# meuleman/epilogos

Measured on AMD Instinct MI355X. Metric: Mbins scored/sec (S1, 18-state, 833 biosamples), higher is better.
Workload: dtype u8

## Files before the change

epilogos_amd/csrc/epg_common.h:

```cpp
#pragma once
#include <hip/hip_runtime.h>
#include <stdarg.h>
#include <stdint.h>
#include <stdio.h>

#include <type_traits>

#include "epilogos_amd.h"

typedef unsigned int u32;
typedef unsigned long long u64;
typedef unsigned short u16;

namespace epg {

int fail(int code, const char* fmt, ...);
int num_cus();

#ifdef EPILOGOS_BUILD_EXPERIMENTS
#include <stdlib.h>
static inline const char* exp_env(const char* name) { return getenv(name); }
#else
static inline const char* exp_env(const char*) { return nullptr; }
#endif

enum Force { FORCE_NULL_SEQ = 0, FORCE_S3_SCORE_BINS, FORCE_S3_CONTRACTION, FORCE_S3_HIST_LDS, FORCE_K1_BLOCKS_PER_CU, FORCE_CUS, FORCE_COUNT };
extern int g_force[FORCE_COUNT];

#define EPG_HIP(expr)                                                                         \
    do {                                                                                      \
        hipError_t _e = (expr);                                                               \
        if (_e != hipSuccess)                                                                 \
            return epg::fail(EPG_ERR_HIP, "%s failed: %s", #expr, hipGetErrorString(_e));     \
    } while (0)

#define EPG_LAUNCH_CHECK(name)                                                                \
    do {                                                                                      \
        hipError_t _e = hipGetLastError();                                                    \
        if (_e != hipSuccess)                                                                 \
            return epg::fail(EPG_ERR_HIP, "launch of %s failed: %s", name, hipGetErrorString(_e)); \
    } while (0)

static inline int64_t align_up(int64_t x, int64_t a) { return (x + a - 1) / a * a; }

template <int DEFAULT, typename F>
static inline auto with_constant(int, F&& f) {
    return f(std::integral_constant<int, DEFAULT>{});
}
template <int DEFAULT, int V, int... VS, typename F>
static inline auto with_constant(int v, F&& f) {
    if (v == V) return f(std::integral_constant<int, V>{});
    return with_constant<DEFAULT, VS...>(v, f);
}

int64_t s1_ws_bytes(int64_t R, int N, int S);
int grid_for_tiles(long R);
long fast_rows(long R, int N, long ldx);
int64_t s2_table_bytes(int maxc, int S);
int64_t s3_ws_bytes(int64_t R, int N, int S);
int64_t s3_xt_bytes(int64_t R, int N);
int transpose_states(const char* X, int64_t R, int32_t N, int64_t ldx, int32_t S, char* XT, int64_t Rp, int shift, int bad, int* dirty,
                     hipStream_t st);
int64_t s3_gemm_ws_bytes(int64_t R, int N, int S);
int64_t s3_gemm_ws_min_bytes(int64_t R, int N, int S);
int hist_s3_gemm(const char* X, int64_t R, int32_t N, int64_t ldx, int32_t S, int32_t* counts, void* ws, int64_t ws_bytes, hipStream_t st);
bool s3_lanes_ok(int N, int S);
int64_t s3_lanes_ws_bytes(int64_t R, int N, int S);
int score_s3_lanes(const int8_t* X8, int64_t R, int32_t N, int64_t ldx, int32_t S, const float* q, double* out64, float* out32, void* ws,
                   int64_t ws_bytes, hipStream_t st);
int wide_hist_s2_from_binhist(const uint16_t* H, const uint16_t* H2, int64_t R, int32_t S, int64_t* counts, hipStream_t st);
int wide_score_s2_from_hist(const uint16_t* H, int64_t R, int32_t S, int64_t perms, const float* q, double* out64, float* out32, hipStream_t st);
int wide_hist_s3(const int8_t* X, int64_t R, int32_t N, int64_t ldx, int32_t S, int32_t* counts, hipStream_t st);
int wide_score_s3(const int8_t* X, int64_t R, int32_t N, int64_t ldx, int32_t S, const float* q, double* out64, float* out32, void* ws,
                  int64_t ws_bytes, hipStream_t st);

struct DynLds {
    unsigned long long done = 0;
};
static inline hipError_t ensure_dyn_lds(DynLds& a, const void* kernel, int bytes) {
    int dev = 0;
    hipError_t e = hipGetDevice(&dev);
    if (e != hipSuccess) return e;
    const unsigned long long bit = 1ull << (dev & 63);
    if (__atomic_load_n(&a.done, __ATOMIC_ACQUIRE) & bit) return hipSuccess;
    e = hipFuncSetAttribute(kernel, hipFuncAttributeMaxDynamicSharedMemorySize, bytes);
    if (e == hipSuccess) __atomic_fetch_or(&a.done, bit, __ATOMIC_RELEASE);
    return e;
}

static inline int tile_rows(int64_t row_bytes) {
    int tr = 64;
    while (tr > 8 && 4 * tr * row_bytes > 65536) tr >>= 1;
    return tr;
}

__device__ __forceinline__ u32 bfi(u32 m, u32 a, u32 b) { return (a & m) | (b & ~m); }

__device__ __forceinline__ uint4 ld16(const char* p) {
    uint4 v;
    __builtin_memcpy(&v, p, 16);
    return v;
}

__device__ __forceinline__ u32 quad_sum(u32 v) {
    v += (u32)__builtin_amdgcn_update_dpp(0, (int)v, 0xB1, 0xf, 0xf, false);
    v += (u32)__builtin_amdgcn_update_dpp(0, (int)v, 0x4E, 0xf, 0xf, false);
    return v;
}

__device__ __forceinline__ void store_staged(const char* lds, char* dst, int nbytes, int lane) {
    const int nchunks = nbytes >> 4;
    for (int c = lane; c < nchunks; c += 64)
        *reinterpret_cast<uint4*>(dst + 16 * c) = *reinterpret_cast<const uint4*>(lds + 16 * c);
    const int tail0 = nchunks << 4;
    for (int o = tail0 + 4 * lane; o + 4 <= nbytes; o += 256)
        *reinterpret_cast<u32*>(dst + o) = *reinterpret_cast<const u32*>(lds + o);
    if ((nbytes & 2) && lane == 0) *reinterpret_cast<u16*>(dst + nbytes - 2) = *reinterpret_cast<const u16*>(lds + nbytes - 2);
}

typedef u32 epg_u32x4 __attribute__((ext_vector_type(4)));
__device__ __forceinline__ void store_staged_nt(const char* lds, char* dst, int nbytes, int lane) {
    const int nchunks = nbytes >> 4;
    for (int c = lane; c < nchunks; c += 64)
        __builtin_nontemporal_store(*reinterpret_cast<const epg_u32x4*>(lds + 16 * c), reinterpret_cast<epg_u32x4*>(dst + 16 * c));
    const int tail0 = nchunks << 4;
    for (int o = tail0 + 4 * lane; o + 4 <= nbytes; o += 256)
        __builtin_nontemporal_store(*reinterpret_cast<const u32*>(lds + o), reinterpret_cast<u32*>(dst + o));
    if ((nbytes & 2) && lane == 0) *reinterpret_cast<u16*>(dst + nbytes - 2) = *reinterpret_cast<const u16*>(lds + nbytes - 2);
}

__device__ __forceinline__ double kl_term(double p, double q) {
    if (q == 0.0) return 0.0;
    const double r = p / q;
    if (!(r > 0.0)) return 0.0;
    return p * log2(r);
}

__device__ __forceinline__ float s3_table_entry(float qv, float obs) {
    if (qv == 0.0f) return 0.0f;
    const float r = __fdiv_rn(obs, qv);
    if (!(r > 0.0f)) return 0.0f;
#ifdef EPG_S3_TABLE_LOG2F
    return obs * log2f(r);
#else
    return __fmul_rn(obs, (float)log2((double)r));
#endif
}

}
```

epilogos_amd/csrc/epg_count.h:

```cpp
#pragma once
#include "epg_common.h"
#include "epg_parts.h"

namespace epg {

#define EPG_B3(a, b, c, tt) ((u32)__builtin_amdgcn_bitop3_b32((int)(a), (int)(b), (int)(c), (tt)))

__device__ __forceinline__ u32 sel(u32 m, u32 x, u32 y) { return EPG_B3(m, x, y, 0xCA); }

__device__ __forceinline__ u32 dbl(u32 x) {
    u32 r;
    asm("v_add_u32 %0, %1, %1" : "=v"(r) : "v"(x));
    return r;
}

__device__ __forceinline__ void bit_planes(const u32 (&w)[8], u32 (&P)[5]) {
    const u32 n0 = sel(0x0f0f0f0fu, w[0], w[1] << 4);
    const u32 n1 = sel(0x0f0f0f0fu, w[2], w[3] << 4);
    const u32 n2 = sel(0x0f0f0f0fu, w[4], w[5] << 4);
    const u32 n3 = sel(0x0f0f0f0fu, w[6], w[7] << 4);
    const u32 m0 = sel(0x33333333u, n0, n1 << 2), m1 = sel(0x33333333u, n2, n3 << 2);
    const u32 r0 = sel(0xccccccccu, n1, n0 >> 2), r1 = sel(0xccccccccu, n3, n2 >> 2);
    P[0] = sel(0x55555555u, m0, dbl(m1)); P[1] = sel(0xaaaaaaaau, m1, m0 >> 1);
    P[2] = sel(0x55555555u, r0, dbl(r1)); P[3] = sel(0xaaaaaaaau, r1, r0 >> 1);
    const u32 c00 = sel(0x10101010u, w[0], dbl(w[4])), c01 = sel(0x10101010u, w[1], dbl(w[5]));
    const u32 c10 = sel(0x10101010u, w[2], dbl(w[6])), c11 = sel(0x10101010u, w[3], dbl(w[7]));
    const u32 d0 = sel(0x30303030u, c00, c10 << 2), d1 = sel(0x30303030u, c01, c11 << 2);
    P[4] = sel(0xf0f0f0f0u, d1, d0 >> 4);
}

__device__ __forceinline__ void low_three(const u32 (&P)[5], u32 (&L)[8]) {
    L[0] = EPG_B3(P[0], P[1], P[2], 0x01); L[1] = EPG_B3(P[0], P[1], P[2], 0x10); L[2] = EPG_B3(P[0], P[1], P[2], 0x04); L[3] = EPG_B3(P[0], P[1], P[2], 0x40);
    L[4] = EPG_B3(P[0], P[1], P[2], 0x02); L[5] = EPG_B3(P[0], P[1], P[2], 0x20); L[6] = EPG_B3(P[0], P[1], P[2], 0x08); L[7] = EPG_B3(P[0], P[1], P[2], 0x80);
}

__device__ __forceinline__ u32 indicator(const u32 (&L)[8], const u32 (&P)[5], int s) {
    switch (s >> 3) {
        case 0: return EPG_B3(L[s & 7], P[3], P[4], 0x10);
        case 1: return EPG_B3(L[s & 7], P[3], P[4], 0x40);
        case 2: return EPG_B3(L[s & 7], P[3], P[4], 0x20);
        default: return EPG_B3(L[s & 7], P[3], P[4], 0x80);
    }
}

template <int S>
__device__ __forceinline__ void count_group(const u32 (&w)[8], u32 (&cnt)[S]) {
    u32 P[5], L[8];
    bit_planes(w, P);
    low_three(P, L);
#pragma unroll
    for (int s = 0; s < S; ++s) cnt[s] += (u32)__builtin_popcount(indicator(L, P, s));
}

struct RowGeom {
    int chunks;
    int last;
    u32 tail[4];
};

__device__ __forceinline__ RowGeom make_geom(int N) {
    RowGeom g;
    g.chunks = (N + 15) >> 4;
    g.last = g.chunks - 1;
    const int t = N - 16 * g.last;
#pragma unroll
    for (int d = 0; d < 4; ++d) {
        int v = t - 4 * d;
        v = v < 0 ? 0 : (v > 4 ? 4 : v);
        g.tail[d] = v == 4 ? 0u : (0xffffffffu << (8 * v));
    }
    return g;
}

template <bool MAYBE_TAIL>
__device__ __forceinline__ void load_slot(const char* rowp, int i, int j, const RowGeom& g, u32* w) {
    const int c = 4 * i + j;
    if (!MAYBE_TAIL) {
        const uint4 v = ld16(rowp + 16 * c);
        w[0] = v.x; w[1] = v.y; w[2] = v.z; w[3] = v.w;
    } else {
        const int cc = c < g.last ? c : g.last;
        const uint4 v = ld16(rowp + 16 * cc);
        const u32 inv = c > g.last ? 0xffffffffu : 0u;
        const bool is_last = c == g.last;
        w[0] = v.x | inv | (is_last ? g.tail[0] : 0u);
        w[1] = v.y | inv | (is_last ? g.tail[1] : 0u);
        w[2] = v.z | inv | (is_last ? g.tail[2] : 0u);
        w[3] = v.w | inv | (is_last ? g.tail[3] : 0u);
    }
}

template <bool MAYBE_TAIL>
__device__ __forceinline__ void load_group(const char* rowp, int t, int j, const RowGeom& g, u32 (&w)[8]) {
    load_slot<MAYBE_TAIL>(rowp, 2 * t, j, g, &w[0]);
    load_slot<MAYBE_TAIL>(rowp, 2 * t + 1, j, g, &w[4]);
}

template <int NG>
__device__ __forceinline__ void load_groups(const char* rowp, int j, const RowGeom& g, u32 (&w)[NG][8]) {
#pragma unroll
    for (int t = 0; t < NG; ++t) {
        if (t < NG - 1) load_group<false>(rowp, t, j, g, w[t]);
        else load_group<true>(rowp, t, j, g, w[t]);
    }
}

template <int NC, typename Group>
__device__ __forceinline__ void for_each_group(const char* rowp, int j, const RowGeom& g, u32 (&cnt)[NC], Group group) {
    const int ngroups = (g.chunks + 7) >> 3;
    for (int t0 = 0; t0 < ngroups; t0 += 4) {
        u32 w[4][8];
#pragma unroll
        for (int k = 0; k < 4; ++k) {
            const int t = t0 + k;
            if (t < ngroups - 1) load_group<false>(rowp, t, j, g, w[k]);
            else if (t == ngroups - 1) load_group<true>(rowp, t, j, g, w[k]);
        }
#pragma unroll
        for (int k = 0; k < 4; ++k)
            if (t0 + k < ngroups) group(t0 + k, w[k], cnt);
    }
}

template <int S, int NG>
__device__ __forceinline__ void count_row(const char* rowp, int j, const RowGeom& g, u32 (&cnt)[S]) {
    if constexpr (NG > 0) {
        u32 w[NG][8];
        load_groups<NG>(rowp, j, g, w);
#pragma unroll
        for (int t = 0; t < NG; ++t) count_group<S>(w[t], cnt);
    } else {
        for_each_group(rowp, j, g, cnt, [](int, const u32 (&w)[8], u32 (&c)[S]) { count_group<S>(w, c); });
    }
}

template <int S, int NG>
struct CountRow {
    __device__ __forceinline__ void operator()(const char* rowp, int j, const RowGeom& g, u32 (&cnt)[S]) const { count_row<S, NG>(rowp, j, g, cnt); }
};

template <int S, typename Count, typename Epilogue, typename Finish>
__device__ __forceinline__ void super_tile(const char* __restrict__ X, long R, long ldx, const RowGeom& g, long lst, int j, int b, Count&& count,
                                           Epilogue&& epilogue, Finish&& finish) {
#pragma unroll
    for (int half = 0; half < 2; ++half) {
        const long row = lst * 32 + half * 16 + b;
        const bool valid = row < R;
        u32 cnt[S];
#pragma unroll
        for (int s = 0; s < S; ++s) cnt[s] = 0;
        count(X + (valid ? row : R - 1) * ldx, j, g, cnt);
        epilogue(half, row, valid, cnt);
    }
    const long row0 = lst * 32;
    finish(lst, row0, (int)(R - row0 < 32 ? R - row0 : 32));
}

template <int S, int NG, int NW = 4, typename Epilogue, typename Finish, typename Count = CountRow<S, NG>>
__device__ __forceinline__ void tile_loop(const char* __restrict__ X, long R, int N, long ldx, Epilogue&& epilogue, Finish&& finish,
                                          Count&& count = Count()) {
    const int lane = threadIdx.x & 63;
    const int wave = __builtin_amdgcn_readfirstlane(threadIdx.x >> 6);
    const int j = lane & 3, b = lane >> 2;
    const RowGeom g = make_geom(N);
    const long nsuper = (R + 31) >> 5;
    for (long st = (long)blockIdx.x * NW + wave; st < nsuper; st += (long)gridDim.x * NW)
        super_tile<S>(X, R, ldx, g, st, j, b, count, epilogue, finish);
}

constexpr int KH_MAXP = 48;
struct KhParts {
    const char* x[KH_MAXP];
    u16* h[KH_MAXP];
    long rows[KH_MAXP];
    long ldx[KH_MAXP];
    long t0[KH_MAXP + 1];
    int n_cols[KH_MAXP];
    int n;
};

template <int S, int NG, int NW = 4, typename Enter, typename Epilogue, typename Finish>
__device__ __forceinline__ void tile_loop_parts(const KhParts& pt, Enter&& enter, Epilogue&& epilogue, Finish&& finish) {
    const int lane = threadIdx.x & 63;
    const int wave = __builtin_amdgcn_readfirstlane(threadIdx.x >> 6);
    const int j = lane & 3, b = lane >> 2;
    const long nsuper = pt.t0[pt.n];
    PartCursor at;
    int part = -1;
    const char* X = nullptr;
    long R = 0, ldx = 0, base = 0;
    RowGeom g = make_geom(16);
    for (long st = (long)blockIdx.x * NW + wave; st < nsuper; st += (long)gridDim.x * NW) {
        at.advance(pt.t0, st, 32);
        if (at.part != part) {
            part = at.part;
            X = pt.x[part];
            R = pt.rows[part];
            ldx = pt.ldx[part];
            base = pt.t0[part];
            g = make_geom(pt.n_cols[part]);
            enter(part);
        }
        super_tile<S>(X, R, ldx, g, st - base, j, b, CountRow<S, NG>(), epilogue, finish);
    }
}

template <int S>
__device__ __forceinline__ void pack_reduce(const u32 (&cnt)[S], u32 (&d)[(S + 1) / 2]) {
#pragma unroll
    for (int m = 0; m < (S + 1) / 2; ++m) {
        const u32 hi = 2 * m + 1 < S ? cnt[2 * m + 1] : 0u;
        d[m] = quad_sum(cnt[2 * m] | (hi << 16));
    }
}

__device__ __forceinline__ u32 sel4(u32 x0, u32 x1, u32 x2, u32 x3, int j) {
    const u32 lo = (j & 1) ? x1 : x0;
    const u32 hi = (j & 1) ? x3 : x2;
    return (j & 2) ? hi : lo;
}

template <int ND>
__device__ __forceinline__ u32 quad_state_count(const u32 (&d)[ND], int k, int j) {
    const u32 lo = d[2 * k], hi = 2 * k + 1 < ND ? d[2 * k + 1] : 0u;
    const u32 v = (j & 2) ? hi : lo;
    return (j & 1) ? v >> 16 : v & 0xffffu;
}

template <int S, bool WHOLE_DWORDS>
__device__ __forceinline__ void stage_hist_row(char* srow, const u32 (&d)[(S + 1) / 2], int j, int Sout) {
    constexpr int ND = (S + 1) / 2;
    if constexpr (WHOLE_DWORDS) {
        static_assert((S & 1) == 0, "whole dwords need an even row");
#pragma unroll
        for (int k = 0; k < (ND + 3) / 4; ++k) {
            const u32 v = sel4(d[4 * k], 4 * k + 1 < ND ? d[4 * k + 1] : 0u, 4 * k + 2 < ND ? d[4 * k + 2] : 0u, 4 * k + 3 < ND ? d[4 * k + 3] : 0u, j);
            if (4 * k + j < ND) *reinterpret_cast<u32*>(srow + 4 * (4 * k + j)) = v;
        }
    } else {
#pragma unroll
        for (int k = 0; k < (S + 3) / 4; ++k) {
            const u32 c = quad_state_count(d, k, j);
            if (4 * k + j < Sout) *reinterpret_cast<u16*>(srow + 2 * (4 * k + j)) = (u16)c;
        }
    }
}

template <int S>
struct StateTotals {
    static constexpr int ND = (S + 1) / 2;
    u32 accp[ND];
    int since, flush_every;
    __device__ __forceinline__ void init(int nmax) {
#pragma unroll
        for (int m = 0; m < ND; ++m) accp[m] = 0;
        flush_every = 65535 / nmax > 1 ? 65535 / nmax - 1 : 1;
        since = 0;
    }
    __device__ __forceinline__ void flush(u64* s_cnt, int j) {
        if (j == 0) {
#pragma unroll
            for (int m = 0; m < ND; ++m) {
                const u32 lo = accp[m] & 0xffffu, hi = accp[m] >> 16;
                if (lo) atomicAdd(&s_cnt[2 * m], (u64)lo);
                if (hi) atomicAdd(&s_cnt[2 * m + 1], (u64)hi);
            }
        }
#pragma unroll
        for (int m = 0; m < ND; ++m) accp[m] = 0;
        since = 0;
    }
    __device__ __forceinline__ void add(const u32 (&d)[ND], bool valid, u64* s_cnt, int j) {
#pragma unroll
        for (int m = 0; m < ND; ++m) accp[m] += valid ? d[m] : 0u;
        if (++since >= flush_every) flush(s_cnt, j);
    }
    __device__ __forceinline__ void commit(u64* s_cnt, int j, u64* __restrict__ counts, int Sout) {
        flush(s_cnt, j);
        __syncthreads();
        if ((int)threadIdx.x < Sout && s_cnt[threadIdx.x]) atomicAdd(&counts[threadIdx.x], s_cnt[threadIdx.x]);
    }
};

}
```

epilogos_amd/csrc/epg_s1.hip:

```cpp
#include "epg_count.h"
#include "epg_paircount.h"

#include <stdlib.h>
#include <string.h>

namespace epg {

constexpr int K1P_LD = 17;

template <int SC, bool FULL, bool PAIRS, typename Loop>
__device__ __forceinline__ void bin_hist_body(int Sout_, u64* __restrict__ counts, int nmax, u64* __restrict__ counts2, Loop&& loop) {
    constexpr int S = SC;
    constexpr int ND = (S + 1) / 2;
    const int Sout = FULL ? S : Sout_;
    const int ROWB = 2 * Sout;
    __shared__ u64 s_cnt[S + 1];
    __shared__ __attribute__((aligned(16))) char s_stage[4][32 * 2 * S];
    constexpr int PG = (S + 2) / 3, PSP = 3 * PG, PROLES = PG * (PG + 1) / 2, PSLICE = PROLES <= 64 ? 64 / PROLES : 1;
    static_assert(!PAIRS || (FULL && PROLES <= 64), "the pair counts need a compile-time row width and at most 64 block roles");
    __shared__ u32 s_pair[PAIRS ? 4 * PSP * K1P_LD : 1];
    __shared__ u64 s_c2[PAIRS ? S * S : 1];
    const int lane = threadIdx.x & 63, wave = threadIdx.x >> 6;
    const int j = lane & 3, b = lane >> 2;
    if (threadIdx.x <= S) s_cnt[threadIdx.x] = 0;
    if (PAIRS) {
        for (int e = threadIdx.x; e < S * S; e += 256) s_c2[e] = 0;
        for (int e = threadIdx.x; e < 4 * PSP * K1P_LD; e += 256) s_pair[e] = 0;
    }
    __syncthreads();
    u16* H = nullptr;
    int pgi = -1, pgj = 0, pkq = 0;
    u64 pacc[PAIRS ? 9 : 1], prs[PAIRS ? 3 : 1];
    if (PAIRS) {
        const int role = lane < PROLES * PSLICE ? lane / PSLICE : -1;
        pkq = lane % PSLICE;
        if (role >= 0) pair_role(role, PG, pgi, pgj);
#pragma unroll
        for (int c = 0; c < 9; ++c) pacc[c] = 0;
#pragma unroll
        for (int c = 0; c < 3; ++c) prs[c] = 0;
    }
    auto pair_counts = [&](const char* stage, int rows) {
        u32* sp = s_pair + wave * PSP * K1P_LD;
        const u16* raw = reinterpret_cast<const u16*>(stage);
        __builtin_amdgcn_wave_barrier();
        for (int e = lane; e < S * 16; e += 64) {
            const int i = e >> 4, k = e & 15;
            const u32 lo = 2 * k < rows ? raw[(2 * k) * S + i] : 0u, hi = 2 * k + 1 < rows ? raw[(2 * k + 1) * S + i] : 0u;
            sp[i * K1P_LD + k] = lo | (hi << 16);
        }
        __builtin_amdgcn_wave_barrier();
        if (pgi >= 0) {
            u32 part[9], ps[3];
            pair_tile_dot(sp + 3 * pgi * K1P_LD, sp + 3 * pgj * K1P_LD, K1P_LD, pkq, 16, PSLICE, pgi == pgj, part, ps);
#pragma unroll
            for (int c = 0; c < 9; ++c) pacc[c] += part[c];
#pragma unroll
            for (int c = 0; c < 3; ++c) prs[c] += ps[c];
        }
        __builtin_amdgcn_wave_barrier();
    };

    StateTotals<S> totals;
    totals.init(nmax);

    auto enter = [&](u16* Hpart) { H = Hpart; };
    auto epilogue = [&](int half, long row, bool valid, u32 (&cnt)[S]) {
        u32 d[ND];
        pack_reduce<S>(cnt, d);
        if (counts) totals.add(d, valid, s_cnt, j);
        if (H) stage_hist_row<S, FULL && (S & 1) == 0>(&s_stage[wave][(half * 16 + b) * ROWB], d, j, Sout);
    };
    auto finish = [&](long st, long row0, int rows) {
        if (H) store_staged(s_stage[wave], reinterpret_cast<char*>(H) + row0 * ROWB, rows * ROWB, lane);
        if constexpr (PAIRS) pair_counts(s_stage[wave], rows);
    };
    loop(enter, epilogue, finish);

    if (counts) totals.commit(s_cnt, j, counts, Sout);
    if constexpr (PAIRS) {
        if (pgi >= 0) pair_fold(pacc, prs, pgi, pgj, S, s_c2);
        pair_commit(s_c2, S, counts2);
    }
}

template <int SC, int NG, bool FULL>
__global__ __launch_bounds__(256) void k_bin_hist(const char* __restrict__ X, long R, int N, long ldx, int Sout_,
                                                   u16* __restrict__ H, u64* __restrict__ counts) {
    bin_hist_body<SC, FULL, false>(Sout_, counts, N, nullptr, [&](auto&& enter, auto&& epilogue, auto&& finish) {
        enter(H);
        tile_loop<SC, NG>(X, R, N, ldx, epilogue, finish);
    });
}

template <int SC, int NG>
__global__ __launch_bounds__(256) void k_bin_hist_s2(const char* __restrict__ X, long R, int N, long ldx, u16* __restrict__ H,
                                                      u64* __restrict__ counts, u64* __restrict__ counts2) {
    bin_hist_body<SC, true, true>(SC, counts, N, counts2, [&](auto&& enter, auto&& epilogue, auto&& finish) {
        enter(H);
        tile_loop<SC, NG>(X, R, N, ldx, epilogue, finish);
    });
}

template <int SC, int NG, bool FULL>
__global__ __launch_bounds__(256) void k_bin_hist_parts(const KhParts pt, int Sout_, u64* __restrict__ counts, int nmax) {
    bin_hist_body<SC, FULL, false>(Sout_, counts, nmax, nullptr, [&](auto&& enter, auto&& epilogue, auto&& finish) {
        tile_loop_parts<SC, NG>(pt, [&](int part) { enter(pt.h[part]); }, epilogue, finish);
    });
}

__global__ __launch_bounds__(256) void k_bin_hist_safe(const char* __restrict__ X, long row_begin, long row_end, int N,
                                                        long ldx, int S, u16* __restrict__ H, u64* __restrict__ counts, int mask = 31) {
    __shared__ u32 s_h[4][128];
    const int lane = threadIdx.x & 63, wave = threadIdx.x >> 6;
    for (long row = row_begin + (long)blockIdx.x * 4 + wave; row < row_end; row += (long)gridDim.x * 4) {
        for (int s = lane; s < S; s += 64) s_h[wave][s] = 0;
        __builtin_amdgcn_wave_barrier();
        const char* rp = X + row * ldx;
        for (int n = lane; n < N; n += 64) {
            const int v = (unsigned char)rp[n] & mask;
            if (v < S) atomicAdd(&s_h[wave][v], 1u);
        }
        __builtin_amdgcn_wave_barrier();
        for (int s = lane; s < S; s += 64) {
            const u32 c = s_h[wave][s];
            if (H) H[row * S + s] = (u16)c;
            if (counts && c) atomicAdd(&counts[s], (u64)c);
        }
        __builtin_amdgcn_wave_barrier();
    }
}

__global__ void k_s1_table(const float* __restrict__ q, int N, int S, double* __restrict__ T64, float* __restrict__ T32) {
    const long e = (long)blockIdx.x * blockDim.x + threadIdx.x;
    if (e >= (long)(N + 1) * S) return;
    const int c = (int)(e / S), s = (int)(e % S);
    const double p = (double)c / (double)N;
    const double v = kl_term(p, (double)q[s]);
    T64[e] = v;
    T32[e] = (float)v;
}

template <int S, int NG, typename OT>
__global__ __launch_bounds__(256) void k_score_s1(const char* __restrict__ X, long R, int N, long ldx,
                                                   const OT* __restrict__ T, OT* __restrict__ out) {
    constexpr int ND = (S + 1) / 2;
    constexpr int ROWB = S * (int)sizeof(OT);
    __shared__ __attribute__((aligned(16))) char s_stage[4][32 * ROWB];
    const int lane = threadIdx.x & 63, wave = threadIdx.x >> 6;
    const int j = lane & 3, b = lane >> 2;
    auto epilogue = [&](int half, long row, bool valid, u32 (&cnt)[S]) {
        u32 d[ND];
        pack_reduce<S>(cnt, d);
        OT* srow = reinterpret_cast<OT*>(&s_stage[wave][(half * 16 + b) * ROWB]);
#pragma unroll
        for (int k = 0; k < (S + 3) / 4; ++k) {
            const u32 c = quad_state_count(d, k, j);
            const int s = 4 * k + j;
            if (s < S) srow[s] = (c && valid) ? T[(long)c * S + s] : (OT)0;
        }
    };
    auto finish = [&](long st, long row0, int rows) {
        store_staged_nt(s_stage[wave], reinterpret_cast<char*>(out) + row0 * ROWB, rows * ROWB, lane);
    };
    tile_loop<S, NG>(X, R, N, ldx, epilogue, finish);
}

template <typename OT, bool LDS_T>
__global__ __launch_bounds__(LDS_T ? 1024 : 256) void k_score_s1_from_hist(const u16* __restrict__ H, long total, int S,
                                                                             const OT* __restrict__ Tg, int nent, OT* __restrict__ out,
                                                                             u64* __restrict__ zero_counts, int rev) {
    extern __shared__ __attribute__((aligned(16))) char smem_t[];
    if (zero_counts && blockIdx.x == 0 && (int)threadIdx.x < S) zero_counts[threadIdx.x] = 0;
    const OT* T = Tg;
    if (LDS_T) {
        OT* Ts = reinterpret_cast<OT*>(smem_t);
        for (int e = threadIdx.x; e < nent; e += blockDim.x) Ts[e] = Tg[e];
        __syncthreads();
        T = Ts;
    }
    const u32 cmax = (u32)(nent / S - 1);
    const long nquads = total >> 2;
    const long stride = (long)gridDim.x * blockDim.x;
    long qd = (long)blockIdx.x * blockDim.x + threadIdx.x;
    const long qtop = nquads - 1, qsgn = rev ? -1 : 1, qoff = rev ? qtop : 0;
    for (; qd + 3 * stride < nquads; qd += 4 * stride) {
        uint2 h[4];
#pragma unroll
        for (int u = 0; u < 4; ++u) h[u] = *reinterpret_cast<const uint2*>(H + 4 * (qoff + qsgn * (qd + u * stride)));
#pragma unroll
        for (int u = 0; u < 4; ++u) {
            const long e0 = 4 * (qoff + qsgn * (qd + u * stride));
            int s = (int)(e0 % S);
            const u32 c[4] = {h[u].x & 0xffffu, h[u].x >> 16, h[u].y & 0xffffu, h[u].y >> 16};
            OT v[4];
#pragma unroll
            for (int k = 0; k < 4; ++k) {
                v[k] = c[k] - 1u < cmax ? T[(long)c[k] * S + s] : (OT)0;
                s = s + 1 == S ? 0 : s + 1;
            }
            if constexpr (sizeof(OT) == 4) {
                typedef float v4f_nt __attribute__((ext_vector_type(4)));
                const v4f_nt vv = {(float)v[0], (float)v[1], (float)v[2], (float)v[3]};
                __builtin_nontemporal_store(vv, reinterpret_cast<v4f_nt*>(out + e0));
            } else {
                typedef double v2d_nt __attribute__((ext_vector_type(2)));
                const v2d_nt lo = {(double)v[0], (double)v[1]}, hi = {(double)v[2], (double)v[3]};
                __builtin_nontemporal_store(lo, reinterpret_cast<v2d_nt*>(out + e0));
                __builtin_nontemporal_store(hi, reinterpret_cast<v2d_nt*>(out + e0 + 2));
            }
        }
    }
    for (; qd < nquads; qd += stride) {
        const long e0 = 4 * (qoff + qsgn * qd);
        int s = (int)(e0 % S);
        for (int k = 0; k < 4; ++k) {
            const u32 c = H[e0 + k];
            out[e0 + k] = c - 1u < cmax ? T[(long)c * S + s] : (OT)0;
            s = s + 1 == S ? 0 : s + 1;
        }
    }
    if (blockIdx.x == 0 && threadIdx.x < (total & 3)) {
        const long e = (nquads << 2) + threadIdx.x;
        const u32 c = H[e];
        out[e] = c - 1u < cmax ? T[(long)c * S + (int)(e % S)] : (OT)0;
    }
}

template <typename IT>
__global__ __launch_bounds__(256) void k_sum_int(const IT* __restrict__ C, long n, long long* __restrict__ total) {
    long long acc = 0;
    for (long i = (long)blockIdx.x * blockDim.x + threadIdx.x; i < n; i += (long)gridDim.x * blockDim.x) acc += (long long)C[i];
    for (int off = 32; off > 0; off >>= 1) acc += __shfl_down(acc, off);
    __shared__ long long s_part[4];
    if ((threadIdx.x & 63) == 0) s_part[threadIdx.x >> 6] = acc;
    __syncthreads();
    if (threadIdx.x == 0) {
        const long long t = s_part[0] + s_part[1] + s_part[2] + s_part[3];
        if (t) atomicAdd(reinterpret_cast<u64*>(total), (u64)t);
    }
}

template <typename IT>
__global__ __launch_bounds__(256) void k_normalise(const IT* __restrict__ C, long n, const long long* __restrict__ total,
                                                    float* __restrict__ q) {
    const double tot = (double)(*total);
    for (long i = (long)blockIdx.x * blockDim.x + threadIdx.x; i < n; i += (long)gridDim.x * blockDim.x)
        q[i] = (float)((double)C[i] / tot);
}

template <typename IT>
__global__ __launch_bounds__(256) void k_normalise_small(const IT* __restrict__ C, int n, float* __restrict__ q) {
    __shared__ long long s_part[4];
    long long acc = 0;
    for (int i = threadIdx.x; i < n; i += 256) acc += (long long)C[i];
    for (int off = 32; off > 0; off >>= 1) acc += __shfl_down(acc, off);
    if ((threadIdx.x & 63) == 0) s_part[threadIdx.x >> 6] = acc;
    __syncthreads();
    const double tot = (double)(s_part[0] + s_part[1] + s_part[2] + s_part[3]);
    for (int i = threadIdx.x; i < n; i += 256) q[i] = (float)((double)C[i] / tot);
}

static int blocks_per_cu() { return g_force[FORCE_K1_BLOCKS_PER_CU] > 0 ? g_force[FORCE_K1_BLOCKS_PER_CU] : 2; }
int grid_for_tiles(long R) {
    const long nsuper = (R + 31) >> 5;
    long blocks = (nsuper + 3) / 4;
    const long cap = (long)num_cus() * blocks_per_cu();
    if (blocks > cap) {
        const long iters = (nsuper + cap * 4 - 1) / (cap * 4);
        blocks = (nsuper + iters * 4 - 1) / (iters * 4);
    }
    if (blocks < 1) blocks = 1;
    return (int)blocks;
}

template <typename F>
static void with_count_core(int S, int ng, F&& f) {
    if (S == 15 || S == 18 || S == 25)
        with_constant<25, 15, 18>(S, [&](auto sc) {
            with_constant<0, 1, 2, 3, 4, 5, 6, 7, 8>(ng, [&](auto NG) { f(sc, NG, std::true_type{}); });
        });
    else
        with_constant<31, 15, 18, 25>(S < 15 ? 15 : S < 18 ? 18 : S < 25 ? 25 : 31,
                                      [&](auto sc) { f(sc, std::integral_constant<int, 0>{}, std::false_type{}); });
}

long fast_rows(long R, int N, long ldx) {
    const long chunks = (N + 15) / 16;
    const long over = 16 * chunks - ldx;
    if (over <= 0) return R;
    const long unsafe = (over + ldx - 1) / ldx;
    return R > unsafe ? R - unsafe : 0;
}

extern "C" int epg_bin_hist(const int8_t* X8, int64_t R, int32_t N, int64_t ldx, int32_t S, uint16_t* H, int64_t* counts, void* stream) {
    hipStream_t st = (hipStream_t)stream;
    if (R < 0 || N < 1 || ldx < N || S < 1) return fail(EPG_ERR_INVALID_ARG, "bin_hist: bad shape R=%lld N=%d ldx=%lld S=%d", (long long)R, N, (long long)ldx, S);
    if (S > 127) return fail(EPG_ERR_UNSUPPORTED, "bin_hist: S=%d > 127 (states are int8)", S);
    if (N > 65535) return fail(EPG_ERR_UNSUPPORTED, "bin_hist: N=%d > 65535 (uint16 per-bin counts)", N);
    if (R == 0) return EPG_OK;
    if (!X8) return fail(EPG_ERR_INVALID_ARG, "bin_hist: X is NULL");
    if (H && (reinterpret_cast<uintptr_t>(H) & 15)) return fail(EPG_ERR_INVALID_ARG, "bin_hist: H must be 16-byte aligned");
    const char* X = reinterpret_cast<const char*>(X8);
    u64* cnt = reinterpret_cast<u64*>(counts);
    if (S > 31) {
        hipLaunchKernelGGL(k_bin_hist_safe, dim3((unsigned)((R + 3) / 4 < num_cus() * 32L ? (R + 3) / 4 : num_cus() * 32L)), dim3(256), 0, st, X, 0L,
                           (long)R, N, ldx, S, H, cnt, 255);
        EPG_LAUNCH_CHECK("k_bin_hist_safe");
        return EPG_OK;
    }
    const long Rf = fast_rows(R, N, ldx);
    if (Rf > 0) {
        with_count_core(S, (N + 127) / 128, [&](auto SC, auto NG, auto MODEL) {
            hipLaunchKernelGGL((k_bin_hist<SC, NG, MODEL && (SC & 1) == 0>), dim3(grid_for_tiles(Rf)), dim3(256), 0, st, X, Rf, N, ldx, S, H, cnt);
        });
        EPG_LAUNCH_CHECK("k_bin_hist");
    }
    if (Rf < R) {
        hipLaunchKernelGGL(k_bin_hist_safe, dim3((unsigned)((R - Rf + 3) / 4 < 1024 ? (R - Rf + 3) / 4 : 1024)), dim3(256), 0, st, X, Rf, (long)R, N, ldx, S, H, cnt);
        EPG_LAUNCH_CHECK("k_bin_hist_safe");
    }
    return EPG_OK;
}

extern "C" int epg_bin_hist_s2(const int8_t* X8, int64_t R, int32_t N, int64_t ldx, int32_t S, uint16_t* H, int64_t* counts, int64_t* counts2,
                               void* stream) {
    hipStream_t st = (hipStream_t)stream;
    if (!H || !counts2) return fail(EPG_ERR_INVALID_ARG, "bin_hist_s2: H and counts2 are required");
    const bool fused = (S == 15 || S == 18 || S == 25) && R > 0 && N >= 1 && N <= 1024 && ldx >= N && X8 &&
                       !(reinterpret_cast<uintptr_t>(H) & 15) && fast_rows(R, N, ldx) == R;
    if (!fused) {
        int rc = epg_bin_hist(X8, R, N, ldx, S, H, counts, stream);
        if (rc) return rc;
        return epg_hist_s2_from_binhist(H, R, S, counts2, stream);
    }
    const char* X = reinterpret_cast<const char*>(X8);
    u64* c1 = reinterpret_cast<u64*>(counts);
    u64* c2 = reinterpret_cast<u64*>(counts2);
    with_constant<25, 18, 15>(S, [&](auto SC) {
        with_constant<8, 1, 2, 3, 4, 5, 6, 7>((N + 127) / 128, [&](auto NG) {
            hipLaunchKernelGGL((k_bin_hist_s2<decltype(SC)::value, NG>), dim3(grid_for_tiles(R)), dim3(256), 0, st, X, R, N, ldx, H, c1, c2);
        });
    });
    EPG_LAUNCH_CHECK("k_bin_hist_s2");
    return EPG_OK;
}

extern "C" int epg_bin_hist_parts(int32_t nparts, const int8_t* const* X, const int64_t* R, const int32_t* N, const int64_t* ldx, int32_t S,
                                  uint16_t* const* H, int64_t* counts, void* stream) {
    hipStream_t st = (hipStream_t)stream;
    if (nparts < 0 || (nparts && (!X || !R || !N || !ldx))) return fail(EPG_ERR_INVALID_ARG, "bin_hist_parts: NULL argument array");
    if (S < 1 || S > 127) return fail(EPG_ERR_UNSUPPORTED, "bin_hist_parts: S=%d outside 1..127", S);
    for (int p = 0; p < nparts; ++p) {
        if (R[p] < 0 || (R[p] && (N[p] < 1 || ldx[p] < N[p]))) return fail(EPG_ERR_INVALID_ARG, "bin_hist_parts: bad shape of part %d", p);
        if (R[p] && N[p] > 65535) return fail(EPG_ERR_UNSUPPORTED, "bin_hist_parts: N=%d > 65535 (uint16 per-bin counts)", N[p]);
        if (R[p] && !X[p]) return fail(EPG_ERR_INVALID_ARG, "bin_hist_parts: X of part %d is NULL", p);
        if (H && H[p] && (reinterpret_cast<uintptr_t>(H[p]) & 15)) return fail(EPG_ERR_INVALID_ARG, "bin_hist_parts: H of part %d must be 16-byte aligned", p);
    }
    if (S > 31) {
        for (int p = 0; p < nparts; ++p) {
            const int rc = epg_bin_hist(X[p], R[p], N[p], ldx[p], S, H ? H[p] : nullptr, counts, stream);
            if (rc) return rc;
        }
        return EPG_OK;
    }
    u64* cnt = reinterpret_cast<u64*>(counts);
    for (int p = 0; p < nparts; ++p) {
        const long Rf = R[p] ? fast_rows(R[p], N[p], ldx[p]) : 0;
        if (Rf == R[p]) continue;
        hipLaunchKernelGGL(k_bin_hist_safe, dim3((unsigned)((R[p] - Rf + 3) / 4 < 1024 ? (R[p] - Rf + 3) / 4 : 1024)), dim3(256), 0, st,
                           reinterpret_cast<const char*>(X[p]), Rf, (long)R[p], N[p], (long)ldx[p], S, H ? H[p] : nullptr, cnt);
        EPG_LAUNCH_CHECK("k_bin_hist_safe");
    }
    auto cls = [](int n) { const int ng = (n + 127) / 128; return ng <= 8 ? ng : 0; };
    for (int c = 0; c <= 8; ++c) {
        for (int p0 = 0; p0 < nparts;) {
            KhParts pt;
            int nmax = 1;
            p0 = pack_parts(pt, p0, nparts, 32, [&](int p) { return R[p] && cls(N[p]) == c ? fast_rows(R[p], N[p], ldx[p]) : 0L; },
                            [&](int k, int p) {
                                pt.x[k] = reinterpret_cast<const char*>(X[p]); pt.h[k] = H ? H[p] : nullptr;
                                pt.ldx[k] = ldx[p]; pt.n_cols[k] = N[p];
                                if (N[p] > nmax) nmax = N[p];
                            });
            if (pt.n == 0) break;
            with_count_core(S, c, [&](auto SC, auto NG, auto) {
                hipLaunchKernelGGL((k_bin_hist_parts<SC, NG, (NG > 0 && (SC & 1) == 0)>), dim3(grid_for_tiles(pt.t0[pt.n] * 32)), dim3(256), 0, st, pt, S,
                                   cnt, nmax);
            });
            EPG_LAUNCH_CHECK("k_bin_hist_parts");
        }
    }
    return EPG_OK;
}

static int64_t s1_table_bytes(int N, int S) { return align_up((int64_t)(N + 1) * S * 8, 256) + align_up((int64_t)(N + 1) * S * 4, 256); }

int64_t s1_ws_bytes(int64_t R, int N, int S) {
    return s1_table_bytes(N, S) + 256 + align_up(R * S * 2, 256);
}

static int build_s1_table(const float* q, int N, int S, void* ws, double** T64, float** T32, hipStream_t st) {
    *T64 = reinterpret_cast<double*>(ws);
    *T32 = reinterpret_cast<float*>(reinterpret_cast<char*>(ws) + align_up((int64_t)(N + 1) * S * 8, 256));
    const long n = (long)(N + 1) * S;
    hipLaunchKernelGGL(k_s1_table, dim3((int)((n + 255) / 256)), dim3(256), 0, st, q, N, S, *T64, *T32);
    EPG_LAUNCH_CHECK("k_s1_table");
    return EPG_OK;
}
static int check_score_from_hist_args(const uint16_t* H, const double* out64, const float* out32) {
    if ((reinterpret_cast<uintptr_t>(H) & 7) != 0) return fail(EPG_ERR_INVALID_ARG, "score_s1_from_binhist: H must be 8-byte aligned");
    if ((out32 && (reinterpret_cast<uintptr_t>(out32) & 15)) || (out64 && (reinterpret_cast<uintptr_t>(out64) & 15)))
        return fail(EPG_ERR_INVALID_ARG, "score_s1_from_binhist: outputs must be 16-byte aligned");
    return EPG_OK;
}

template <typename OT>
static int launch_score_s1_from_hist_t(const uint16_t* H, long total, int32_t S, const OT* T, int nent, OT* out, u64* zero_counts, hipStream_t st) {
    const size_t tbytes = (size_t)nent * sizeof(OT);
    const int rev = 1;
    if (tbytes <= 150 * 1024) {
        const int per_cu = tbytes <= 75 * 1024 ? 2 : 1;
        long nb = (total / 4 + 4095) / 4096;
        if (nb > (long)num_cus() * per_cu) nb = (long)num_cus() * per_cu;
        if (nb < 1) nb = 1;
        auto kern = k_score_s1_from_hist<OT, true>;
        static DynLds lds_attr;
        EPG_HIP(ensure_dyn_lds(lds_attr, reinterpret_cast<const void*>(kern), 150 * 1024));
        hipLaunchKernelGGL(kern, dim3((int)nb), dim3(1024), tbytes, st, H, total, S, T, nent, out, zero_counts, rev);
    } else {
        long nb = (total / 4 + 1023) / 1024;
        if (nb > num_cus() * 8L) nb = num_cus() * 8L;
        if (nb < 1) nb = 1;
        hipLaunchKernelGGL((k_score_s1_from_hist<OT, false>), dim3((int)nb), dim3(256), 0, st, H, total, S, T, nent, out, zero_counts, rev);
    }
    EPG_LAUNCH_CHECK("k_score_s1_from_hist");
    return EPG_OK;
}

static int launch_score_s1_from_hist(const uint16_t* H, int64_t R, int32_t N, int32_t S, const double* T64, const float* T32,
                                     double* out64, float* out32, hipStream_t st, u64* zero_counts = nullptr) {
    const long total = (long)R * S;
    const int nent = (N + 1) * S;
    int rc = EPG_OK;
    if (out32) rc = launch_score_s1_from_hist_t<float>(H, total, S, T32, nent, out32, zero_counts, st);
    if (!rc && out64) rc = launch_score_s1_from_hist_t<double>(H, total, S, T64, nent, out64, out32 ? nullptr : zero_counts, st);
    return rc;
}


extern "C" int epg_score_s1_from_binhist(const uint16_t* H, int64_t R, int32_t N, int32_t S, const float* q, double* out64, float* out32,
                                         void* ws, int64_t ws_bytes, void* stream) {
    hipStream_t st = (hipStream_t)stream;
    if (R < 0 || N < 1 || S < 1) return fail(EPG_ERR_INVALID_ARG, "score_s1: bad shape");
    if (R == 0) return EPG_OK;
    if (!H || !q || !ws) return fail(EPG_ERR_INVALID_ARG, "score_s1_from_binhist: NULL argument");
    if (ws_bytes < s1_table_bytes(N, S)) return fail(EPG_ERR_WORKSPACE, "score_s1: workspace %lld < %lld bytes", (long long)ws_bytes, (long long)s1_table_bytes(N, S));
    int rc = check_score_from_hist_args(H, out64, out32);
    if (rc) return rc;
    double* T64; float* T32;
    rc = build_s1_table(q, N, S, ws, &T64, &T32, st);
    if (rc) return rc;
    return launch_score_s1_from_hist(H, R, N, S, T64, T32, out64, out32, st);
}

extern "C" int epg_score_s1_from_binhist_table(const uint16_t* H, int64_t R, int32_t N, int32_t S, const double* T64, const float* T32,
                                               double* out64, float* out32, void* stream) {
    if (R < 0 || N < 1 || S < 1) return fail(EPG_ERR_INVALID_ARG, "score_s1: bad shape");
    if (R == 0) return EPG_OK;
    if (!H || (out64 && !T64) || (out32 && !T32)) return fail(EPG_ERR_INVALID_ARG, "score_s1_from_binhist_table: NULL argument");
    if ((T64 && (reinterpret_cast<uintptr_t>(T64) & 7)) || (T32 && (reinterpret_cast<uintptr_t>(T32) & 3)))
        return fail(EPG_ERR_INVALID_ARG, "score_s1_from_binhist_table: misaligned table");
    int rc = check_score_from_hist_args(H, out64, out32);
    if (rc) return rc;
    return launch_score_s1_from_hist(H, R, N, S, T64, T32, out64, out32, (hipStream_t)stream);
}

__global__ __launch_bounds__(256) void k_s1_combine(const u64* __restrict__ counts, int N, int S, float* __restrict__ q,
                                                     double* __restrict__ T64, float* __restrict__ T32) {
    __shared__ long long s_c[128];
    __shared__ double s_q[128];
    const int t = threadIdx.x;
    if (t < S) s_c[t] = (long long)counts[t];
    __syncthreads();
    if (t < S) {
        long long tot = 0;
        for (int s = 0; s < S; ++s) tot += s_c[s];
        const float qf = (float)((double)s_c[t] / (double)tot);
        if (blockIdx.x == 0) q[t] = qf;
        s_q[t] = (double)qf;
    }
    __syncthreads();
    const int e = blockIdx.x * 256 + t;
    if (e < (N + 1) * S) {
        const int c = e / S, s = e - c * S;
        const double v = kl_term((double)c / (double)N, s_q[s]);
        T64[e] = v;
        T32[e] = (float)v;
    }
}

extern "C" int epg_combine_score_s1(int64_t* counts, int32_t rezero, const uint16_t* H, int64_t R, int32_t N, int32_t S, float* q,
                                    double* out64, float* out32, void* ws, int64_t ws_bytes, void* stream) {
    hipStream_t st = (hipStream_t)stream;
    if (R < 0 || N < 1 || S < 1) return fail(EPG_ERR_INVALID_ARG, "combine_score_s1: bad shape R=%lld N=%d S=%d", (long long)R, N, S);
    if (S > 127) return fail(EPG_ERR_UNSUPPORTED, "combine_score_s1: S=%d > 127 (states are int8)", S);
    if (!counts || !q || !ws || (R > 0 && !H)) return fail(EPG_ERR_INVALID_ARG, "combine_score_s1: NULL argument");
    if (ws_bytes < s1_table_bytes(N, S)) return fail(EPG_ERR_WORKSPACE, "combine_score_s1: workspace %lld < %lld bytes", (long long)ws_bytes, (long long)s1_table_bytes(N, S));
    int rc = check_score_from_hist_args(H, out64, out32);
    if (rc) return rc;
    double* T64 = reinterpret_cast<double*>(ws);
    float* T32 = reinterpret_cast<float*>(reinterpret_cast<char*>(ws) + align_up((int64_t)(N + 1) * S * 8, 256));
    const long nent = (long)(N + 1) * S;
    hipLaunchKernelGGL(k_s1_combine, dim3((unsigned)((nent + 255) / 256)), dim3(256), 0, st, reinterpret_cast<const u64*>(counts), N, S, q, T64, T32);
    EPG_LAUNCH_CHECK("k_s1_combine");
    if (R == 0 || (!out32 && !out64)) {
        if (rezero) EPG_HIP(hipMemsetAsync(counts, 0, (size_t)S * 8, st));
        return EPG_OK;
    }
    return launch_score_s1_from_hist(H, R, N, S, T64, T32, out64, out32, st, rezero ? reinterpret_cast<u64*>(counts) : nullptr);
}

extern "C" int epg_hist_s1(const int8_t* X, int64_t R, int32_t N, int64_t ldx, int32_t S, int64_t* counts, void* stream) {
    if (!counts) return fail(EPG_ERR_INVALID_ARG, "hist_s1: counts is NULL");
    return epg_bin_hist(X, R, N, ldx, S, nullptr, counts, stream);
}

extern "C" int epg_score_s1(const int8_t* X8, int64_t R, int32_t N, int64_t ldx, int32_t S, const float* q, double* out64, float* out32,
                            void* ws, int64_t ws_bytes, void* stream) {
    hipStream_t st = (hipStream_t)stream;
    if (R < 0 || N < 1 || ldx < N || S < 1) return fail(EPG_ERR_INVALID_ARG, "score_s1: bad shape");
    if (S > 127) return fail(EPG_ERR_UNSUPPORTED, "score_s1: S=%d > 127 (states are int8)", S);
    if (R == 0) return EPG_OK;
    if (!X8 || !q || !ws) return fail(EPG_ERR_INVALID_ARG, "score_s1: NULL argument");
    if ((out32 && (reinterpret_cast<uintptr_t>(out32) & 15)) || (out64 && (reinterpret_cast<uintptr_t>(out64) & 15)))
        return fail(EPG_ERR_INVALID_ARG, "score_s1: outputs must be 16-byte aligned");
    const long Rf = fast_rows(R, N, ldx);
    const bool fused = S == 18 && Rf == R;
    if (!fused) {
        if (ws_bytes < s1_ws_bytes(R, N, S)) return fail(EPG_ERR_WORKSPACE, "score_s1: workspace %lld < %lld bytes", (long long)ws_bytes, (long long)s1_ws_bytes(R, N, S));
        u16* H = reinterpret_cast<u16*>(reinterpret_cast<char*>(ws) + s1_table_bytes(N, S));
        int rc = epg_bin_hist(X8, R, N, ldx, S, H, nullptr, stream);
        if (rc) return rc;
        return epg_score_s1_from_binhist(H, R, N, S, q, out64, out32, ws, s1_table_bytes(N, S), stream);
    }
    if (ws_bytes < s1_table_bytes(N, S)) return fail(EPG_ERR_WORKSPACE, "score_s1: workspace %lld < %lld bytes", (long long)ws_bytes, (long long)s1_table_bytes(N, S));
    double* T64; float* T32;
    int rc = build_s1_table(q, N, S, ws, &T64, &T32, st);
    if (rc) return rc;
    const char* X = reinterpret_cast<const char*>(X8);
    with_constant<0, 1, 2, 3, 4, 5, 6, 7, 8>((N + 127) / 128, [&](auto NG) {
        if (out32) hipLaunchKernelGGL((k_score_s1<18, NG, float>), dim3(grid_for_tiles(R)), dim3(256), 0, st, X, R, N, ldx, T32, out32);
        if (out64) hipLaunchKernelGGL((k_score_s1<18, NG, double>), dim3(grid_for_tiles(R)), dim3(256), 0, st, X, R, N, ldx, T64, out64);
    });
    EPG_LAUNCH_CHECK("k_score_s1");
    return EPG_OK;
}

template <typename IT>
static int normalise_impl(const IT* C, int64_t n, float* q, void* ws, int64_t ws_bytes, hipStream_t st) {
    if (n < 1 || !C || !q || !ws) return fail(EPG_ERR_INVALID_ARG, "normalise: bad argument");
    if (ws_bytes < 8) return fail(EPG_ERR_WORKSPACE, "normalise: workspace needs 8 bytes");
    if (n <= 4096) {
        hipLaunchKernelGGL((k_normalise_small<IT>), dim3(1), dim3(256), 0, st, C, (int)n, q);
        EPG_LAUNCH_CHECK("k_normalise_small");
        return EPG_OK;
    }
    long long* total = reinterpret_cast<long long*>(ws);
    EPG_HIP(hipMemsetAsync(total, 0, 8, st));
    long blocks = (n + 255) / 256;
    if (blocks > num_cus() * 8L) blocks = num_cus() * 8L;
    hipLaunchKernelGGL((k_sum_int<IT>), dim3((int)blocks), dim3(256), 0, st, C, (long)n, total);
    hipLaunchKernelGGL((k_normalise<IT>), dim3((int)blocks), dim3(256), 0, st, C, (long)n, total, q);
    EPG_LAUNCH_CHECK("k_normalise");
    return EPG_OK;
}

extern "C" int epg_normalise_i64(const int64_t* C, int64_t n, float* q, void* ws, int64_t ws_bytes, void* stream) {
    return normalise_impl<long long>(reinterpret_cast<const long long*>(C), n, q, ws, ws_bytes, (hipStream_t)stream);
}
extern "C" int epg_normalise_i32(const int32_t* C, int64_t n, float* q, void* ws, int64_t ws_bytes, void* stream) {
    return normalise_impl<int>(C, n, q, ws, ws_bytes, (hipStream_t)stream);
}

}
```

Measured before the change: 5784.

## Stream bin-hist rows into an LDS ring with async global-to-LDS DMA

Adds a DMA path for the fast bin-histogram kernel. Each wave issues global_load_lds copies of the next 16-row half-tile into its own LDS slot while it counts the current one, then reads the data back with ds_read_b128. This double-buffers memory loads against the popcount work and so hides global load latency. It needs dynamic LDS sized by N, aligned X and ldx, and inline asm waits, and it is used only when the row geometry allows it.

```diff
diff --git a/epilogos_amd/csrc/epg_common.h b/epilogos_amd/csrc/epg_common.h
--- a/epilogos_amd/csrc/epg_common.h
+++ b/epilogos_amd/csrc/epg_common.h
@@ -24,7 +24,8 @@
 static inline const char* exp_env(const char*) { return nullptr; }
 #endif
 
-enum Force { FORCE_NULL_SEQ = 0, FORCE_S3_SCORE_BINS, FORCE_S3_CONTRACTION, FORCE_S3_HIST_LDS, FORCE_K1_BLOCKS_PER_CU, FORCE_CUS, FORCE_COUNT };
+enum Force { FORCE_NULL_SEQ = 0, FORCE_S3_SCORE_BINS, FORCE_S3_CONTRACTION, FORCE_S3_HIST_LDS, FORCE_K1_BLOCKS_PER_CU, FORCE_CUS,
+             FORCE_K1_PLAIN_LOADS, FORCE_COUNT };
 extern int g_force[FORCE_COUNT];
 
 #define EPG_HIP(expr)                                                                         \
diff --git a/epilogos_amd/csrc/epg_count.h b/epilogos_amd/csrc/epg_count.h
--- a/epilogos_amd/csrc/epg_count.h
+++ b/epilogos_amd/csrc/epg_count.h
@@ -166,6 +166,119 @@
     const long nsuper = (R + 31) >> 5;
     for (long st = (long)blockIdx.x * NW + wave; st < nsuper; st += (long)gridDim.x * NW)
         super_tile<S>(X, R, ldx, g, st, j, b, count, epilogue, finish);
+}
+
+typedef u32 epg_ldsx4 __attribute__((ext_vector_type(4)));
+
+template <int NG>
+struct DmaHalfTile {
+    static constexpr int NI = 2 * NG;
+    u32 soff[NI];
+    u64 rpack;
+    char* slot;
+    u32 rd, rd_tail[2];
+    int npieces;
+
+    __device__ __forceinline__ void init(char* ring, int wave, int lane, const RowGeom& g, long ldx) {
+        const int j = lane & 3, b = lane >> 2, C = g.chunks;
+        npieces = 16 * C;
+        slot = ring + wave * (256 * C);
+        rpack = 0;
+#pragma unroll
+        for (int i = 0; i < NI; ++i) {
+            const int p = 64 * i + lane;
+            int r = p / C;
+            const int c = p - r * C;
+            const bool used = r < 16;
+            r = used ? r : 0;
+            soff[i] = used ? (u32)r * (u32)ldx + 16u * (u32)c : 0u;
+            rpack |= (u64)r << (4 * i);
+        }
+        const u32 row = (u32)(uintptr_t)slot + 16u * (u32)(b * C);
+        rd = row + 16u * j;
+#pragma unroll
+        for (int k = 0; k < 2; ++k) {
+            const int c = 4 * (NI - 2 + k) + j;
+            rd_tail[k] = row + 16u * (u32)(c < g.last ? c : g.last);
+        }
+    }
+
+    __device__ __forceinline__ void fill(const char* __restrict__ X, long R, long ldx, long row0, int lane) const {
+        const char* Xh = X + row0 * ldx;
+        const long left = R - row0;
+        auto piece = [&](int i, const char* src) {
+            if (i < NI - 2 || 64 * i + lane < npieces)
+                __builtin_amdgcn_global_load_lds((const __attribute__((address_space(1))) void*)src,
+                                                 (__attribute__((address_space(3))) void*)(slot + 1024 * i), 16, 0, 2 );
+        };
+        if (left >= 16) {
+#pragma unroll
+            for (int i = 0; i < NI; ++i) piece(i, Xh + soff[i]);
+        } else {
+#pragma unroll
+            for (int i = 0; i < NI; ++i) piece(i, (long)((rpack >> (4 * i)) & 15) < left ? Xh + soff[i] : X);
+        }
+    }
+
+    static __device__ __forceinline__ void wait() { asm volatile("s_waitcnt vmcnt(0)" ::: "memory"); }
+
+    __device__ __forceinline__ void read(const RowGeom& g, int j, u32 (&w)[NG][8]) const {
+        epg_ldsx4 v[NI];
+        __builtin_amdgcn_sched_barrier(0);
+#pragma unroll
+        for (int i = 0; i < NI - 2; ++i) asm volatile("ds_read_b128 %0, %1 offset:%2" : "=v"(v[i]) : "v"(rd), "n"(64 * i) : "memory");
+        asm volatile("ds_read_b128 %0, %1" : "=v"(v[NI - 2]) : "v"(rd_tail[0]) : "memory");
+        asm volatile("ds_read_b128 %0, %1" : "=v"(v[NI - 1]) : "v"(rd_tail[1]) : "memory");
+#pragma unroll
+        for (int i = 0; i < NI; ++i) asm volatile("s_waitcnt lgkmcnt(0)" : "+v"(v[i])::"memory");
+        __builtin_amdgcn_sched_barrier(0);
+#pragma unroll
+        for (int i = 0; i < NI; ++i) {
+            u32* o = &w[i >> 1][4 * (i & 1)];
+            o[0] = v[i].x; o[1] = v[i].y; o[2] = v[i].z; o[3] = v[i].w;
+            if (i >= NI - 2) {
+                const int c = 4 * i + j;
+                const u32 inv = c > g.last ? 0xffffffffu : 0u;
+                const bool is_last = c == g.last;
+#pragma unroll
+                for (int d = 0; d < 4; ++d) o[d] |= inv | (is_last ? g.tail[d] : 0u);
+            }
+        }
+    }
+};
+
+template <int S, int NG, int NW = 4, typename Epilogue, typename Finish>
+__device__ __forceinline__ void tile_loop_dma(const char* __restrict__ X, long R, int N, long ldx, char* ring, Epilogue&& epilogue, Finish&& finish) {
+    const int lane = threadIdx.x & 63;
+    const int wave = __builtin_amdgcn_readfirstlane(threadIdx.x >> 6);
+    const int j = lane & 3, b = lane >> 2;
+    const RowGeom g = make_geom(N);
+    const long nsuper = (R + 31) >> 5, stride = (long)gridDim.x * NW;
+    long st = (long)blockIdx.x * NW + wave;
+    if (st >= nsuper) return;
+    DmaHalfTile<NG> dma;
+    dma.init(ring, wave, lane, g, ldx);
+    dma.fill(X, R, ldx, st * 32, lane);
+    dma.wait();
+    for (; st < nsuper; st += stride) {
+#pragma unroll
+        for (int half = 0; half < 2; ++half) {
+            const long row = st * 32 + half * 16 + b;
+            u32 w[NG][8];
+            dma.read(g, j, w);
+            if (half == 0) dma.fill(X, R, ldx, st * 32 + 16, lane);
+            else if (st + stride < nsuper) dma.fill(X, R, ldx, (st + stride) * 32, lane);
+            u32 cnt[S];
+#pragma unroll
+            for (int s = 0; s < S; ++s) cnt[s] = 0;
+#pragma unroll
+            for (int t = 0; t < NG; ++t) count_group<S>(w[t], cnt);
+            dma.wait();
+            epilogue(half, row, row < R, cnt);
+        }
+        const long row0 = st * 32;
+        finish(st, row0, (int)(R - row0 < 32 ? R - row0 : 32));
+    }
 }
 
 constexpr int KH_MAXP = 48;
diff --git a/epilogos_amd/csrc/epg_s1.hip b/epilogos_amd/csrc/epg_s1.hip
--- a/epilogos_amd/csrc/epg_s1.hip
+++ b/epilogos_amd/csrc/epg_s1.hip
@@ -84,12 +84,14 @@
     }
 }
 
-template <int SC, int NG, bool FULL>
+template <int SC, int NG, bool FULL, bool DMA = false>
 __global__ __launch_bounds__(256) void k_bin_hist(const char* __restrict__ X, long R, int N, long ldx, int Sout_,
                                                    u16* __restrict__ H, u64* __restrict__ counts) {
+    extern __shared__ __attribute__((aligned(16))) char s_ring[];
     bin_hist_body<SC, FULL, false>(Sout_, counts, N, nullptr, [&](auto&& enter, auto&& epilogue, auto&& finish) {
         enter(H);
-        tile_loop<SC, NG>(X, R, N, ldx, epilogue, finish);
+        if constexpr (DMA) tile_loop_dma<SC, NG>(X, R, N, ldx, s_ring, epilogue, finish);
+        else tile_loop<SC, NG>(X, R, N, ldx, epilogue, finish);
     });
 }
 
@@ -283,6 +285,10 @@
     else
         with_constant<31, 15, 18, 25>(S < 15 ? 15 : S < 18 ? 18 : S < 25 ? 25 : 31,
                                       [&](auto sc) { f(sc, std::integral_constant<int, 0>{}, std::false_type{}); });
+}
+
+static bool dma_rows_ok(const char* X, long ldx) {
+    return !g_force[FORCE_K1_PLAIN_LOADS] && ((reinterpret_cast<uintptr_t>(X) | (uintptr_t)ldx) & 15) == 0 && ldx < (1L << 27);
 }
 
 long fast_rows(long R, int N, long ldx) {
@@ -311,9 +317,22 @@
     }
     const long Rf = fast_rows(R, N, ldx);
     if (Rf > 0) {
+        hipError_t dyn = hipSuccess;
         with_count_core(S, (N + 127) / 128, [&](auto SC, auto NG, auto MODEL) {
-            hipLaunchKernelGGL((k_bin_hist<SC, NG, MODEL && (SC & 1) == 0>), dim3(grid_for_tiles(Rf)), dim3(256), 0, st, X, Rf, N, ldx, S, H, cnt);
+            constexpr bool FULL = MODEL && (SC & 1) == 0;
+            if constexpr (MODEL && NG > 0) {
+                if (dma_rows_ok(X, ldx)) {
+                    static DynLds lds;
+                    const int ring = 1024 * ((N + 15) / 16);
+                    dyn = ensure_dyn_lds(lds, reinterpret_cast<const void*>(k_bin_hist<SC, NG, FULL, true>), 1024 * 8 * NG);
+                    if (dyn == hipSuccess)
+                        hipLaunchKernelGGL((k_bin_hist<SC, NG, FULL, true>), dim3(grid_for_tiles(Rf)), dim3(256), ring, st, X, Rf, N, ldx, S, H, cnt);
+                    return;
+                }
+            }
+            hipLaunchKernelGGL((k_bin_hist<SC, NG, FULL>), dim3(grid_for_tiles(Rf)), dim3(256), 0, st, X, Rf, N, ldx, S, H, cnt);
         });
+        if (dyn != hipSuccess) return fail(EPG_ERR_HIP, "bin_hist: the LDS ring was refused: %s", hipGetErrorString(dyn));
         EPG_LAUNCH_CHECK("k_bin_hist");
     }
     if (Rf < R) {
```

After: 5976, median of 6. 3.3% higher.
